# Nathan494326/Husky-Rover-MPPI-IsaacSim

Hardware: AMD Instinct MI355X
Metric: MPPI steps/sec at K=65536 H=100 on 750x750 costmap; 1/2/4/8-GPU scaling (higher is better)
Workload: dtype f32

## Files before the change

### husky-rover-mppi-isaacsim_amd/csrc/mppi_kernels.hip

```cpp
#include <hip/hip_runtime.h>

#include <algorithm>
#include <type_traits>
#include <stdint.h>

#include "mppi_detmath.h"
#include "mppi_kernels.h"

namespace mppi {

constexpr bool kFastMath = false;
constexpr bool kChainFast = true;

struct Recip {
  float b, y;
};
__device__ __forceinline__ bool div_ok(float v) {
  const float a = fabsf(v);
  return a >= 9.094947017729282e-13f && a <= 1.099511627776e12f;
}
template <bool F>
__device__ __forceinline__ Recip rc(float b, bool& bad) {
  Recip r;
  r.b = b;
// ... 330 lines not shown
}

struct Head {
  f2 xy;
  float z;
};

template <bool F>
__device__ __forceinline__ Head orient_step(f2 nxy, float nz, const Head& h, float sn, float cs, float omc,
                                           Lean& l) {
  const f2 hn = h.xy * nxy;
  const float d = (hn.x + hn.y) + h.z * nz;
  const f2 pxy = h.xy - bc2(d) * nxy;
  const float pz = h.z - d * nz;
  f2 txy, oxy;
  float tz, oz;
  if constexpr (F) {
    const f2 p2 = pxy * pxy;
    const Recip r = lean_norm2((p2.x + p2.y) + pz * pz, l);
    lean_div3<2>(pxy, pz, r, l, txy, tz);
    const f2 t2 = txy * txy;
    const Recip ro = norm_near1_trusted((t2.x + t2.y) + tz * tz);
    lean_div3<0>(txy, tz, ro, l, oxy, oz);
  } else {
    const float pn = sqrtf((pxy.x * pxy.x + pxy.y * pxy.y) + pz * pz);
    txy = f2{pxy.x / pn, pxy.y / pn};
    tz = pz / pn;
    const float tn = sqrtf((txy.x * txy.x + txy.y * txy.y) + tz * tz);
    oxy = f2{txy.x / tn, txy.y / tn};
    oz = tz / tn;
  }
  const f2 cxy = cross_xy(nxy, nz, oxy, oz);
  const f2 cz2 = nxy * oxy.yx;
  const float crz = cz2.x - cz2.y;
  const f2 no = nxy * oxy;
  const float dn = (no.x + no.y) + nz * oz;
  const f2 rxy = (oxy * bc2(cs) + cxy * bc2(sn)) + (nxy * bc2(dn)) * bc2(omc);
  const float rz = (oz * cs + crz * sn) + (nz * dn) * omc;
  Head o;
  if constexpr (F) {
    const f2 r2 = rxy * rxy;
    const Recip r = lean_norm_near1((r2.x + r2.y) + rz * rz, l);
    lean_div3<2>(rxy, rz, r, l, o.xy, o.z);
  } else {
    const float rn = sqrtf((rxy.x * rxy.x + rxy.y * rxy.y) + rz * rz);
    o.xy = f2{rxy.x / rn, rxy.y / rn};
    o.z = rz / rn;
  }
  return o;
}
template <bool F, bool GUARD = true>
__device__ __forceinline__ f2 advance_step(const Head& h, float v, float dt, f2 pos, Lean& l) {
  f2 u;
  if constexpr (F) {
    const f2 h2 = h.xy * h.xy;
    if constexpr (GUARD) {
      const Recip r = lean_norm_near1((h2.x + h2.y) + h.z * h.z, l);
      u = lean_div2(h.xy, r, l);
    } else {
      const Recip r = norm_near1_trusted((h2.x + h2.y) + h.z * h.z);
      u = lean_div2<0>(h.xy, r, l);
    }
  } else {
    const float hn = sqrtf((h.xy.x * h.xy.x + h.xy.y * h.xy.y) + h.z * h.z);
    u = f2{h.xy.x / hn, h.xy.y / hn};
  }
  return pos + (u * bc2(v)) * bc2(dt);
}

template <bool F>
__device__ __forceinline__ void wheels3d(const Dem& dem, float off, float x, float y,
                                         const float (&q)[4], float nx, float ny, float nz,
                                         float hx, float hy, float hz, StepOut& o, bool& bad) {
  o.z = bilinear<F>(x, y, q, dem.template rr<F>(), bad);
  const float cx = off * (ny * hz - nz * hy);
  const float cy = off * (nz * hx - nx * hz);
  o.lx = x + cx;
  o.ly = y + cy;
  o.lz = dem.template point<F>(o.lx, o.ly, bad);
  o.rx = x - cx;
  o.ry = y - cy;
  o.rz = dem.template point<F>(o.rx, o.ry, bad);
}

template <bool F>
__device__ __forceinline__ void step2d(const Dem& dem, float dt, float v, float sn, float cs,
                                       Traj& s, StepOut& o, bool& bad) {
  {
    const Recip r = rc<F>(sq<F>((s.hx * s.hx + s.hy * s.hy) + s.hz * s.hz, bad), bad);
    const float ux = dv<F>(s.hx, r, bad), uy = dv<F>(s.hy, r, bad);
    s.x = s.x + (ux * v) * dt;
    s.y = s.y + (uy * v) * dt;
  }
  {
    float nx = cs * s.hx - sn * s.hy;
    float ny = sn * s.hx + cs * s.hy;
    const float nrm = sq<F>(nx * nx + ny * ny, bad);
    if (nrm > 0.0f) {
      const Recip r = rc<F>(nrm, bad);
      nx = dv<F>(nx, r, bad);
      ny = dv<F>(ny, r, bad);
    }
    s.hx = nx;
    s.hy = ny;
    s.hz = 0.0f;
  }
  float q[4];
  dem.template corners<F>(s.x, s.y, q, bad);
  o.z = bilinear<F>(s.x, s.y, q, dem.template rr<F>(), bad);
  o.lx = o.ly = o.lz = o.rx = o.ry = o.rz = 0.0f;
}

template <bool F>
__device__ __forceinline__ float slope_term(float plx, float ply, float plz, float clx, float cly,
                                            float clz, float prx, float pry, float prz, float crx,
                                            float cry, float crz, bool& bad) {
  const float eps = 1e-6f;
  const float dzl = clz - plz;
  const float dxl = clx - plx, dyl = cly - ply;
  const float dl = sq<F>(dxl * dxl + dyl * dyl, bad);
  const float dzr = crz - prz;
  const float dxr = crx - prx, dyr = cry - pry;
  const float dr = sq<F>(dxr * dxr + dyr * dyr, bad);
  const float ratl = fabsf(dv1<F>(dzl, dl + eps, bad));
  const float ratr = fabsf(dv1<F>(dzr, dr + eps, bad));
  const float al = 1.0f + 5.0f * ratl;
  const float ar = 1.0f + 5.0f * ratr;
  const float ls = al * al, rs = ar * ar;
  return (ls > rs) ? ls : rs;
}

template <bool F>
__device__ __forceinline__ int costmap_index(int size, float hw, const Recip& rres_c, float x,
                                             float y, bool& bad, float rinv = 0.0f, int cdiv = 0) {
  float fx, fy;
  if (cdiv) {
    fx = cdiv_f(x + hw, rres_c.b, rinv);
    fy = cdiv_f((-y) + hw, rres_c.b, rinv);
  } else {
    fx = dv<F>(x + hw, rres_c, bad);
    fy = dv<F>((-y) + hw, rres_c, bad);
  }
  const int ix = (int)__builtin_amdgcn_fmed3f(fx, 0.0f, (float)(size - 1));
  const int iy = (int)__builtin_amdgcn_fmed3f(fy, 0.0f, (float)(size - 1));
  return ix + size * iy;
}


__device__ __forceinline__ float wave_min(float v) {
#pragma unroll
  for (int o = 32; o > 0; o >>= 1) v = fminf(v, __shfl_xor(v, o, 64));
  return v;
}

struct __attribute__((aligned(16))) PairScale {
  float m;
  float ea, eb;
  int mode;
};
__device__ __forceinline__ PairScale pair_scale(float ma, float mb, float T) {
  PairScale p;
  const bool ae = !(ma < INFINITY);
  const bool be = !(mb < INFINITY);
  p.m = fminf(ma, mb);
  p.ea = p.eb = 0.0f;
  if (ae) {
    p.mode = 2;
  } else if (be) {
    p.mode = 1;
  } else {
    p.mode = 0;
    p.ea = dm_expf(-((ma - p.m) / T));
    p.eb = dm_expf(-((mb - p.m) / T));
  }
  return p;
}
__device__ __forceinline__ double pair_apply(const PairScale& p, double a, double b, int j) {
  if (p.mode == 1) return a;
  if (p.mode == 2) return b;
  if (j == 0) return (double)p.m;
  return (double)p.ea * a + (double)p.eb * b;
}
__device__ __forceinline__ PairScale ld_scale(const PairScale* ps) { return *ps; }
__device__ __forceinline__ double pair_apply_raw(const PairScale p, double a, double b, int j) {
  double r = (double)p.ea * a + (double)p.eb * b;
  asm volatile("" : "+v"(r));
  const double n = j == 0 ? (double)p.m : r;
  return p.mode == 1 ? a : (p.mode == 2 ? b : n);
}
__device__ __forceinline__ double pair_apply_sel(const PairScale& ps, double a, double b, int j) {
  return pair_apply_raw(ps, a, b, j);
}

template <int G>
__device__ __forceinline__ void group_scales(const float (&m)[G], float T, PairScale (&ps)[G - 1]) {
  float cur[G];
#pragma unroll
  for (int i = 0; i < G; ++i) cur[i] = m[i];
  int base = 0;
#pragma unroll
  for (int w = G / 2; w >= 1; w >>= 1) {
#pragma unroll
    for (int i = 0; i < w; ++i) {
      ps[base + i] = pair_scale(cur[2 * i], cur[2 * i + 1], T);
      cur[i] = ps[base + i].m;
    }
    base += w;
  }
}
template <int G>
__device__ __forceinline__ double group_apply(const PairScale* ps, const double (&v)[G], int j) {
  double cur[G];
#pragma unroll
  for (int i = 0; i < G; ++i) cur[i] = v[i];
  int base = 0;
#pragma unroll
  for (int w = G / 2; w >= 1; w >>= 1) {
#pragma unroll
    for (int i = 0; i < w; ++i) cur[i] = pair_apply(ps[base + i], cur[2 * i], cur[2 * i + 1], j);
    base += w;
  }
  return cur[0];
}

template <bool FRESH, int NT = 1024>
__device__ __forceinline__ int thread_id() {
  int t = threadIdx.x;
  if constexpr (FRESH) asm volatile("" : "+v"(t));
  __builtin_assume(t >= 0 && t < NT);
  return t;
}

struct NoiseVals {
  float a1, a2, b1, b2;
};
__device__ __forceinline__ NoiseVals noise_gen(uint64_t seed, uint64_t n_base, int64_t k_offset, int blk, int n, int tj) {
  const uint64_t kg = (uint64_t)(k_offset + (int64_t)blk * 256 + tj);
  NoiseVals v;
  noise_block_pk(seed, n_base + (uint64_t)n, kg, &v.a1, &v.a2, &v.b1, &v.b2);
  return v;
}
__device__ __forceinline__ void noise_store(float* __restrict__ eps, int H, int blk, int n, int tj, const NoiseVals& v) {
  const int t = 2 * n;
  float* e1 = eps + ((size_t)blk * 2 * H + t) * 256 + tj;
  float* e2 = e1 + (size_t)H * 256;
  __hip_atomic_store(e1, v.a1, __ATOMIC_RELAXED, __HIP_MEMORY_SCOPE_AGENT);
  __hip_atomic_store(e2, v.a2, __ATOMIC_RELAXED, __HIP_MEMORY_SCOPE_AGENT);
  if (t + 1 < H) {
    __hip_atomic_store(e1 + 256, v.b1, __ATOMIC_RELAXED, __HIP_MEMORY_SCOPE_AGENT);
    __hip_atomic_store(e2 + 256, v.b2, __ATOMIC_RELAXED, __HIP_MEMORY_SCOPE_AGENT);
  }
}
__device__ __forceinline__ void noise_unit(uint64_t seed, uint64_t n_base, int64_t k_offset, int H, int blk, int n,
                                           float* __restrict__ eps, int tj) {
  noise_store(eps, H, blk, n, tj, noise_gen(seed, n_base, k_offset, blk, n, tj));
}
__device__ __forceinline__ void noise_rows(uint64_t seed, uint64_t n_base, int64_t k_offset, int H, int end,
                                           float* __restrict__ eps, int g0, int gstride, int tj) {
  const int NB = (H + 1) >> 1;
  if (g0 >= end) return;
  int blk = g0 / NB, n = g0 - blk * NB;
  const int sq = gstride / NB, sr = gstride - sq * NB;
  for (int g = g0; g < end; g += gstride) {
    noise_unit(seed, n_base, k_offset, H, blk, n, eps, tj);
    blk += sq;
    n += sr;
    if (n >= NB) {
      n -= NB;
      ++blk;
    }
  }
}
struct NoisePos {
  int q, g, blk, n;
};
__device__ __forceinline__ void noise_pos_step(NoisePos& p, int stride, int NB) {
  p.q += stride;
  p.n += (p.q >> 2) - p.g;
  p.g = p.q >> 2;
  while (p.n >= NB) {
    p.n -= NB;
    ++p.blk;
  }
}
__device__ __forceinline__ void noise_waves(uint64_t seed, uint64_t n_base, int64_t k_offset, int H, int q, int q1,
                                            int stride, float* __restrict__ eps, int lane) {
  const int NB = (H + 1) >> 1;
  if (q >= q1) return;
  NoisePos a;
  a.q = q;
  a.g = q >> 2;
  a.blk = a.g / NB;
  a.n = a.g - a.blk * NB;
  for (;;) {
    NoisePos b = a;
    noise_pos_step(b, stride, NB);
    const bool has_b = b.q < q1;
    if (!has_b) b = a;
    const NoiseVals va = noise_gen(seed, n_base, k_offset, a.blk, a.n, ((a.q & 3) << 6) + lane);
    const NoiseVals vb = noise_gen(seed, n_base, k_offset, b.blk, b.n, ((b.q & 3) << 6) + lane);
    noise_store(eps, H, a.blk, a.n, ((a.q & 3) << 6) + lane, va);
    if (!has_b) break;
    noise_store(eps, H, b.blk, b.n, ((b.q & 3) << 6) + lane, vb);
    a = b;
    noise_pos_step(a, stride, NB);
    if (a.q >= q1) break;
  }
}

constexpr int UCACHE_ROW = 256 + 4;
template <int TB, int NT, bool EPS = false, bool WT = false>
__device__ __forceinline__ void leaf_records(const RolloutArgs& a, const float* cost_lds,
                                             unsigned char* scratch, const float* ub_block,
                                             const float* unom = nullptr, const float* ucache = nullptr,
                                             int uc_steps = 0, int blk = -1);

template <int TB, int NT, bool EPS, bool WT>
__device__ __forceinline__ void leaf_records(const RolloutArgs& a, const float* cost_lds,
                                             unsigned char* scratch, const float* ub_block,
                                             const float* unom, const float* ucache, int uc_steps, int blk) {
  if (blk < 0) blk = blockIdx.x;
  constexpr int NL = TB / 256;
  constexpr int NWL = TB / 64;
  const int tid = thread_id<WT, NT>(), lane = tid & 63;
  const int wave = __builtin_amdgcn_readfirstlane(tid >> 6);
  const int H = a.H, E = 2 * H + 2;
  float* wbuf = reinterpret_cast<float*>(scratch);
  float* wave_m = wbuf + TB;
  double* red = reinterpret_cast<double*>(scratch + ((TB + NWL) * 4 + 15) / 16 * 16);
  const int NR = NL * (E - 1);
  const int NU = ((NR + 7) >> 3) << 6;
  struct Unit {
    float4 uq[8];
    int j;
    bool cached;
    float nom, sg, lo, hi;
    const float4* w4;
  };
  auto load = [&](int it, Unit& U) __attribute__((always_inline)) {
    const int k = (it >> 3) & 7;
    const int r = min(((it >> 6) << 3) + (it & 7), NR - 1);
    const int half = k >> 2, line = k & 3;
    const int leaf = r / (E - 1), j = 1 + r - leaf * (E - 1);
    U.j = j;
    const int tr0 = 256 * leaf + 128 * half + 32 * line;
    U.w4 = reinterpret_cast<const float4*>(wbuf + tr0);
    const float4* u4 = reinterpret_cast<const float4*>(ub_block + (size_t)(j >= 2 ? j - 2 : 0) * TB + tr0);
    U.cached = false;
    U.nom = U.sg = U.lo = U.hi = 0.f;
    if constexpr (EPS) {
      const int c = (j - 2) >= H ? 1 : 0;
      const int t = max(j - 2, 0) - c * H;
      const int ti = min(t + 1, H - 1);
      U.nom = unom[c * H + ti];
      U.sg = c ? a.s2 : a.s1;
      U.lo = c ? a.min_u2 : a.min_u1;
      U.hi = c ? a.max_u2 : a.max_u1;
      if (j >= 2 && t < uc_steps) {
        U.cached = true;
        u4 = reinterpret_cast<const float4*>(ucache + (size_t)(c * uc_steps + t) * UCACHE_ROW + tr0);
      }
    }
#pragma unroll
    for (int g = 0; g < 8; ++g) U.uq[g] = (j >= 2) ? u4[g] : make_float4(1.f, 1.f, 1.f, 1.f);
  };
  auto reduce = [&](int it, const Unit& U) __attribute__((always_inline)) {
    const int j = U.j;
    double gs[8];
#pragma unroll
    for (int g = 0; g < 8; ++g) {
      const float4 w = U.w4[g];
      float4 u = U.uq[g];
      if (EPS && !U.cached) {
        u.x = clampf(U.nom + U.sg * u.x, U.lo, U.hi);
        u.y = clampf(U.nom + U.sg * u.y, U.lo, U.hi);
        u.z = clampf(U.nom + U.sg * u.z, U.lo, U.hi);
        u.w = clampf(U.nom + U.sg * u.w, U.lo, U.hi);
      }
      if (j < 2) u = make_float4(1.f, 1.f, 1.f, 1.f);
      const double x = __builtin_fma((double)w.x, (double)u.x, (double)w.y * (double)u.y);
      const double y = __builtin_fma((double)w.z, (double)u.z, (double)w.w * (double)u.w);
      gs[g] = x + y;
    }
    const double ls = ((gs[0] + gs[1]) + (gs[2] + gs[3])) + ((gs[4] + gs[5]) + (gs[6] + gs[7]));
    const double s2 = ls + __shfl_xor(ls, 8, 64);
    const double hs = s2 + __shfl_xor(s2, 16, 64);
    const double rs = hs + __shfl_xor(hs, 32, 64);
    const int r = ((it >> 6) << 3) + (it & 7);
    if (r < NR && ((it >> 3) & 7) == 0) {
      const int leaf = r / (E - 1);
      red[leaf * E + j] = rs;
    }
  };
  Unit first;
  if (tid < NU) load(tid, first);
  if (wave < NWL) {
    const float wm = wave_min(cost_lds[tid]);
    if (lane == 0) wave_m[wave] = wm;
  }
  __syncthreads();
  for (int j = tid; j < TB; j += NT) {
    const int leaf = j >> 8;
    const float m = fminf(fminf(wave_m[4 * leaf], wave_m[4 * leaf + 1]),
                          fminf(wave_m[4 * leaf + 2], wave_m[4 * leaf + 3]));
    const float c = cost_lds[j];
    wbuf[j] = (c < INFINITY) ? dm_expf(-((c - m) / a.T)) : 0.0f;
  }
  __syncthreads();
  if (tid < NU) reduce(tid, first);
  for (int it = NT + tid; it < NU; it += NT) {
    Unit U;
    load(it, U);
    reduce(it, U);
  }
  __syncthreads();
  for (int j = tid; j < E; j += NT) {
    double val[NL];
    float lm[NL];
#pragma unroll
    for (int q = 0; q < NL; ++q) {
      lm[q] = fminf(fminf(wave_m[4 * q], wave_m[4 * q + 1]), fminf(wave_m[4 * q + 2], wave_m[4 * q + 3]));
      val[q] = (j == 0) ? (double)lm[q] : red[q * E + j];
    }
#pragma unroll
    for (int width = NL; width > 1; width >>= 1) {
#pragma unroll
      for (int q = 0; q < width / 2; ++q) {
        const PairScale ps = pair_scale(lm[2 * q], lm[2 * q + 1], a.T);
        val[q] = pair_apply(ps, val[2 * q], val[2 * q + 1], j);
        lm[q] = ps.m;
      }
    }
    if constexpr (WT)
      __hip_atomic_store(a.nodes + (size_t)blk * E + j, val[0], __ATOMIC_RELAXED, __HIP_MEMORY_SCOPE_AGENT);
    else
      a.nodes[(size_t)blk * E + j] = val[0];
    if (j == 0 && a.rec_m) {
      if constexpr (WT)
        __hip_atomic_store(a.rec_m + blk, lm[0], __ATOMIC_RELAXED, __HIP_MEMORY_SCOPE_AGENT);
      else
        a.rec_m[blk] = lm[0];
    }
  }
}

constexpr int PAIR_D = PAIR_RING;
constexpr int PAIR_LAG = 4;
static_assert(PAIR_LAG > 0 && PAIR_LAG < PAIR_D, "ring depth must exceed the consume lag");
static_assert(PAIR_LAG % 2 == 0, "the side loop pairs even and odd steps");

__device__ __forceinline__ int lds_load_acquire(const int* f) {
  const int v = __hip_atomic_load(f, __ATOMIC_RELAXED, __HIP_MEMORY_SCOPE_WORKGROUP);
  __builtin_amdgcn_fence(__ATOMIC_ACQUIRE, "workgroup", "local");
  return v;
}
__device__ __forceinline__ void lds_store_release(int* f, int v) {
  __builtin_amdgcn_fence(__ATOMIC_RELEASE, "workgroup", "local");
  __hip_atomic_store(f, v, __ATOMIC_RELAXED, __HIP_MEMORY_SCOPE_WORKGROUP);
}

__device__ __forceinline__ void lds_wait_ge(const int* f, int target, int& seen) {
  if (seen >= target) return;
  int v;
  while ((v = lds_load_acquire(f)) < target) {
  }
  seen = v;
}

template <int TB, int NC, bool DUMP, int DO = PAIR_D>
__device__ __forceinline__ void chain_wave_3d(const RolloutArgs& a, const Dem& dem, const Traj& s, int tj,
                                              bool valid, int64_t kl, const float* ring_in, float* ring_out,
                                              const int* f_prod, int* f_chain, const int* const (&f_cons)[NC],
                                              int& seen_prod, int (&seen_cons)[NC]) {
  constexpr int D = PAIR_D;
  constexpr int RI = 4;
  using T_ = std::true_type;
  using F_ = std::false_type;
  const int H = a.H;
  bool nobad = false;
  const bool clk = a.clk != nullptr && blockIdx.x == 0 && tj < 64;
  uint64_t clk_t0 = 0, clk_r0 = 0;
  if (clk) {
    clk_t0 = __builtin_amdgcn_s_memtime();
    clk_r0 = __builtin_amdgcn_s_memrealtime();
  }
  auto body = [&](auto cd_tag) __attribute__((always_inline)) {
      constexpr bool CD = decltype(cd_tag)::value;
      Head hd{f2{s.hx, s.hy}, s.hz};
      f2 posA = f2{s.x, s.y}, posB = posA;
      float4 nvA = make_float4(0.f, 0.f, 0.f, 0.f), nvB = nvA;
      float snA = 0.f, csA = 0.f, omA = 0.f, snB = 0.f, csB = 0.f, omB = 0.f;
      const f2 cell_off = f2{-a.x_min, a.y_min};
      const float fi_hi = (float)(a.grid - 1), fj_lo = (float)(1 - a.rows);
      const char* nbase = reinterpret_cast<const char*>(dem.N);
      const int nrow = a.grid + 1;
      const int ncol0 = a.grid + 2;
      auto gather = [&](f2 pos, float4& nv) __attribute__((always_inline)) {
        f2 f;
        if constexpr (CD) {
          const f2 aa = pos + cell_off;
          const f2 q0 = aa * bc2(dem.rinv);
          const f2 r = pk_fma(-q0, bc2(dem.res), aa);
          f = pk_fma(r, bc2(dem.rinv), q0);
        } else {
          f = f2{(pos.x - a.x_min) / a.res, (pos.y + a.y_min) / a.res};
        }
        const int ti = (int)__builtin_amdgcn_fmed3f(f.x, -1.0f, fi_hi);
        const int tjj = (int)__builtin_amdgcn_fmed3f(f.y, fj_lo, 1.0f);
        const int idx = __mul24(tjj, -nrow) + (ti + ncol0);
        nv = *reinterpret_cast<const float4*>(nbase + (uint32_t)(idx << 4));
      };
      auto read_in = [&](int t, float& v, float& sn, float& cs, float& om, int need) __attribute__((always_inline)) {
        if (need) lds_wait_ge(f_prod, need, seen_prod);
        const float* ri = ring_in + (t % D) * RI * TB + tj;
        v = ri[0];
        sn = ri[TB];
        cs = ri[2 * TB];
        om = ri[3 * TB];
      };
      {
        float v0;
        read_in(0, v0, snA, csA, omA, 1);
        Lean l;
        lean_init(l);
        f2 p = advance_step<true>(hd, v0, a.dt, posA, l);
        if (__builtin_expect(lean_bad(l), 0)) p = advance_step<false>(hd, v0, a.dt, posA, l);
        posA = p;
        gather(posA, nvA);
      }
      auto it = [&](auto even_tag, auto more_tag, int t, f2& pX, float4& nX, float& snX, float& csX, float& omX,
                    f2& pY, float4& nY, float& snY, float& csY, float& omY) __attribute__((always_inline)) {
        constexpr bool EVEN = decltype(even_tag)::value;
        constexpr bool more = decltype(more_tag)::value;
        float v1 = 0.f;
        if constexpr (more) read_in(t + 1, v1, snY, csY, omY, EVEN ? min(t + 3, H) : 0);
        const f2 nxy = f2{nX.x, nX.y};
        const float nz = nX.z;
        Lean l;
        lean_init(l);
        Head ho = orient_step<true>(nxy, nz, hd, snX, csX, omX, l);
        f2 p1 = pX;
        if constexpr (more) p1 = advance_step<true, false>(ho, v1, a.dt, pX, l);
        if (__builtin_expect(lean_bad(l), 0)) {
          ho = orient_step<false>(nxy, nz, hd, snX, csX, omX, l);
          if constexpr (more) p1 = advance_step<false>(ho, v1, a.dt, pX, l);
        }
        const f2 cxy = bc2(a.off) * cross_xy(nxy, nz, ho.xy, ho.z);
        if constexpr (more) {
          pY = p1;
          gather(pY, nY);
        }
        if constexpr (EVEN) {
#pragma unroll
          for (int c = 0; c < NC; ++c) lds_wait_ge(f_cons[c], t - DO + 2, seen_cons[c]);
        }
        float* ro = ring_out + (t % DO) * 4 * TB + tj;
        ro[0] = pX.x;
        ro[TB] = pX.y;
        ro[2 * TB] = cxy.x;
        ro[3 * TB] = cxy.y;
        if constexpr (DUMP) {
          if (valid) {
            float q[4];
            dem.template corners<false>(pX.x, pX.y, q, nobad);
            const float z = bilinear<false>(pX.x, pX.y, q, dem.template rr<false>(), nobad);
            const size_t o3 = ((size_t)kl * H + t) * 3;
// ... 1839 lines not shown
    bool flagged = false;
    if (what == 0) {
      const float want = a / b;
      const float got = dv1<true>(a, b, flagged);
      if (!flagged && f_bits(want) != f_bits(got)) ++local;
    } else if (what == 1) {
      const float x = fabsf(a);
      const float want = sqrtf(x);
      const float got = sq<true>(x, flagged);
      if (!flagged && f_bits(want) != f_bits(got)) ++local;
    } else {
      const U4 r2 = philox4x32_10(U4{(uint32_t)i, (uint32_t)(i >> 32), 0x5e1fu, 0x1ea4u}, (uint32_t)seed,
                                  (uint32_t)(seed >> 32));
      const float c = (what == 3) ? bits_f((r2.x & 0x807FFFFFu) | ((127u - 30u + r2.y % 60u) << 23))
                                  : mk(r2.x, r2.y);
      const float n = (a * a + b * b) + c * c;
      const float sr = sqrtf(n);
      Lean l;
      lean_init(l);
      const Recip rr = lean_norm(n, l);
      const float g0 = lean_div(a, rr, l), g1 = lean_div(b, rr, l), g2 = lean_div(c, rr, l);
      if (!lean_bad(l) && (f_bits(rr.b) != f_bits(sr) || f_bits(g0) != f_bits(a / sr) ||
                           f_bits(g1) != f_bits(b / sr) || f_bits(g2) != f_bits(c / sr)))
        ++local;
    }
  }
  if (local) atomicAdd(bad_count, local);
}

template <int TB, int PROJ>
static hipError_t launch_pair_m(const RolloutArgs& a, int blocks, size_t lds, hipStream_t st, int mode,
                                bool dump) {
  if (mode == 0) {
    if (dump)
      hipLaunchKernelGGL((mppi_rollout_pair_kernel<TB, PROJ, 0, true>), dim3(blocks), dim3(2 * TB), lds, st, a);
    else
      hipLaunchKernelGGL((mppi_rollout_pair_kernel<TB, PROJ, 0, false>), dim3(blocks), dim3(2 * TB), lds, st, a);
  } else {
    if (dump)
      hipLaunchKernelGGL((mppi_rollout_pair_kernel<TB, PROJ, 1, true>), dim3(blocks), dim3(2 * TB), lds, st, a);
    else
      hipLaunchKernelGGL((mppi_rollout_pair_kernel<TB, PROJ, 1, false>), dim3(blocks), dim3(2 * TB), lds, st, a);
  }
  return hipGetLastError();
}

template <int TB, int PROJ>
static hipError_t launch_roles_m(const RolloutArgs& a, int blocks, size_t lds, hipStream_t st, int mode,
                                 bool dump) {
  const dim3 g(blocks), b(NROLES * TB);
  if (mode == 0) {
    if (dump)
      hipLaunchKernelGGL((mppi_rollout_roles_kernel<TB, PROJ, 0, true>), g, b, lds, st, a);
    else
      hipLaunchKernelGGL((mppi_rollout_roles_kernel<TB, PROJ, 0, false>), g, b, lds, st, a);
  } else {
    if (dump)
      hipLaunchKernelGGL((mppi_rollout_roles_kernel<TB, PROJ, 1, true>), g, b, lds, st, a);
    else
      hipLaunchKernelGGL((mppi_rollout_roles_kernel<TB, PROJ, 1, false>), g, b, lds, st, a);
  }
  return hipGetLastError();
}

hipError_t launch_rollout_pair(const RolloutArgs& a, int blocks, size_t lds, hipStream_t st, int proj,
                               int mode, bool dump, bool roles) {
  if (roles) {
    if (proj == 3) return launch_roles_m<256, 3>(a, blocks, lds, st, mode, dump);
    return launch_roles_m<256, 2>(a, blocks, lds, st, mode, dump);
  }
  if (proj == 3) return launch_pair_m<256, 3>(a, blocks, lds, st, mode, dump);
  return launch_pair_m<256, 2>(a, blocks, lds, st, mode, dump);
}

hipError_t launch_finish(const FinishArgs& f, size_t lds, hipStream_t st, int groups) {
  hipLaunchKernelGGL(mppi_finish_kernel, dim3(groups), dim3(FIN_THREADS), lds, st, f);
  return hipGetLastError();
}

int colfin_shape(int n, int H, int* P_out, int* ncol_out, int* groups_out, size_t* lds_tree, int max_groups) {
  if (n < 1 || n > COLFIN_PMAX || max_groups < 1) return 0;
  int P = 16;
  while (P < n) P *= 2;
  const int E = 2 * H + 2;
  const int ncol = std::max({2, (E + 63) / 64, (E + max_groups - 1) / max_groups});
  if ((ncol + 1) * (P / 16) > FIN_THREADS) return 0;
  const int groups = (E + ncol - 1) / ncol;
  *P_out = P;
  *ncol_out = ncol;
  *groups_out = groups;
  *lds_tree = (size_t)(P - 1) * sizeof(PairScale) + (size_t)(2 * P) * sizeof(float) +
              (size_t)(ncol + 1) * (P / 16) * sizeof(double);
  return 1;
}

hipError_t launch_colfin(const FinishArgs& f, size_t lds, hipStream_t st, int P, int ncol, int groups) {
  hipLaunchKernelGGL(mppi_colfin_kernel, dim3(groups), dim3(FIN_THREADS), lds, st, f, P, ncol);
  return hipGetLastError();
}

hipError_t launch_tail(const FinishArgs& f, hipStream_t st) {
  const size_t lds = (size_t)(12 * f.H + 4) * sizeof(float);
  hipLaunchKernelGGL(mppi_tail_kernel, dim3(1), dim3(TAIL_THREADS), lds, st, f);
  return hipGetLastError();
}

__global__ __launch_bounds__(256) void mppi_normal_table_kernel(const float* __restrict__ Z, int rows, int grid,
                                                                float res, float4* __restrict__ out) {
  const int64_t cols = (int64_t)grid + 1;
  const int64_t n = ((int64_t)rows + 1) * cols;
  const float res_half_neg = (-res) / 2.0f;
  const float res_sq = res * res;
  for (int64_t g = (int64_t)blockIdx.x * 256 + threadIdx.x; g < n; g += (int64_t)gridDim.x * 256) {
    const int j = (int)(g / cols) - 1, i = (int)(g % cols) - 1;
    const int r0 = clampi(j, 0, rows - 1), r1 = clampi(j + 1, 0, rows - 1);
    const int c0 = clampi(i, 0, grid - 1), c1 = clampi(i + 1, 0, grid - 1);
    const float q0 = Z[(size_t)r0 * grid + c0], q1 = Z[(size_t)r0 * grid + c1];
    const float q2 = Z[(size_t)r1 * grid + c0], q3 = Z[(size_t)r1 * grid + c1];
    bool unused = false;
    const float vx = res_half_neg * (((q1 - q0) - q2) + q3);
    const float vy = res_half_neg * (((q2 - q0) - q1) + q3);
    const Recip r = rc<false>(sq<false>((vx * vx + vy * vy) + res_sq * res_sq, unused), unused);
    out[g] = make_float4(dv<false>(vx, r, unused), dv<false>(vy, r, unused), dv<false>(res_sq, r, unused), 0.0f);
  }
}

hipError_t launch_normal_table(const float* Z, int rows, int grid, float res, float4* out, hipStream_t st) {
  const int64_t n = ((int64_t)rows + 1) * ((int64_t)grid + 1);
  const unsigned blocks = (unsigned)std::min<int64_t>((n + 255) / 256, 256 * 16);
  hipLaunchKernelGGL(mppi_normal_table_kernel, dim3(blocks), dim3(256), 0, st, Z, rows, grid, res, out);
  return hipGetLastError();
}

__global__ __launch_bounds__(256) void mppi_noise_kernel(uint64_t seed, uint64_t n_base, int64_t k_offset,
                                                         int H, int n_blocks, float* __restrict__ eps) {
  noise_rows(seed, n_base, k_offset, H, n_blocks * ((H + 1) >> 1), eps, blockIdx.x, gridDim.x, threadIdx.x);
}

struct ServerLaunch {
  RolloutArgs a;
  ServerArgs z;
};
__device__ __forceinline__ const ServerLaunch* fresh_args() {
#if __HIP_DEVICE_COMPILE__
  uint64_t v = reinterpret_cast<uint64_t>(__builtin_amdgcn_kernarg_segment_ptr());
  asm volatile("" : "+s"(v));
  return (const ServerLaunch*)reinterpret_cast<const __attribute__((address_space(4))) ServerLaunch*>(v);
#else
  return nullptr;
#endif
}

template <int TB, int PROJ>
__global__ __launch_bounds__(NROLES * TB) void mppi_step_server_kernel(const ServerLaunch args) {
  __shared__ unsigned cmd_lds[32];
  __shared__ int sh[2];
  const int tid = threadIdx.x;
  unsigned expect = args.z.first_seq;
  bool head = blockIdx.x == 0;
  for (;;) {
    const auto* L = fresh_args();
    const ServerArgs& z = L->z;
    if (tid < 64) {
      const int slot = tid < kCmdWords ? tid : 0;
      const unsigned long long* src =
          (head ? reinterpret_cast<const unsigned long long*>(z.cmd->slot) : z.relay) + slot;
      const unsigned* host_stop = reinterpret_cast<const unsigned*>(z.cmd->slot + kCmdStopSlot);
      unsigned ok = 0;
      unsigned long long w = 0;
      const uint64_t t0 = __builtin_amdgcn_s_memrealtime();
      uint64_t t_stop = t0;
      if (tid == 0 && head && z.clk) z.clk[kClkServer + 8 * (expect & 7) + 6] = t0;
      const bool forced = head && z.exit_after != 0 && expect - z.first_seq >= z.exit_after;
      while (!forced) {
        w = head ? __hip_atomic_load(src, __ATOMIC_RELAXED, __HIP_MEMORY_SCOPE_SYSTEM)
                 : __hip_atomic_load(src, __ATOMIC_RELAXED, __HIP_MEMORY_SCOPE_AGENT);
        const unsigned lo = (unsigned)w, hi = (unsigned)(w >> 32);
        const unsigned long long stop_slot = (unsigned)__builtin_amdgcn_readlane((int)lo, kCmdStopSlot);
        if (cmd_stop_hit(stop_slot, z.launch_id)) break;
        const unsigned seq0 = (unsigned)__builtin_amdgcn_readfirstlane((int)hi);
        if (__builtin_amdgcn_ballot_w64(!cmd_slot_ok(slot, w, seq0, expect)) == 0) {
          ok = 1;
          break;
        }
        const uint64_t now = __builtin_amdgcn_s_memrealtime();
        if (head) {
          if (now - t0 >= z.idle_ticks) break;
        } else {
          if (now - t_stop >= 10000) {
            t_stop = now;
            if (__hip_atomic_load(host_stop, __ATOMIC_RELAXED, __HIP_MEMORY_SCOPE_SYSTEM) == z.launch_id) break;
          }
          __builtin_amdgcn_s_sleep(2);
        }
      }
      if (ok && tid < kCmdWords) {
        if (head && tid != kCmdStopSlot)
          __hip_atomic_store(z.relay + tid, w, __ATOMIC_RELAXED, __HIP_MEMORY_SCOPE_AGENT);
        cmd_lds[tid] = (unsigned)w;
      }
      if (head && !ok && tid == 0)
        __hip_atomic_store(z.relay + kCmdStopSlot, (unsigned long long)z.launch_id, __ATOMIC_RELAXED,
                           __HIP_MEMORY_SCOPE_AGENT);
      if (tid == 0) cmd_lds[31] = ok;
      if (tid == 0 && head && z.clk && ok)
        __hip_atomic_store(z.clk + kClkServer + 8 * (cmd_lds[0] & 7), (uint64_t)__builtin_amdgcn_s_memrealtime(),
                           __ATOMIC_RELAXED, __HIP_MEMORY_SCOPE_AGENT);
    }
    __syncthreads();
    if (!cmd_lds[31]) return;
    const ServerCmd& c = *reinterpret_cast<const ServerCmd*>(cmd_lds);
    auto rd = [&](const float& x) __attribute__((always_inline)) {
      return __builtin_bit_cast(float, __builtin_amdgcn_readfirstlane(__builtin_bit_cast(int, x)));
    };
    const unsigned seq = __builtin_amdgcn_readfirstlane(c.seq);
    const int eps_slot = __builtin_amdgcn_readfirstlane(c.eps_slot);
    const int cur = __builtin_amdgcn_readfirstlane(c.cur);
    RolloutArgs a = L->a;
    a.eps = z.eps[eps_slot];
    a.u_nom1 = z.u_nom[cur];
    a.u_nom2 = z.u_nom[cur] + a.H;
    a.x0 = rd(c.x0);
    a.y0 = rd(c.y0);
    a.h0x = rd(c.h0x);
    a.h0y = rd(c.h0y);
    a.h0z = rd(c.h0z);
    a.wl = rd(c.wl);
    a.wr = rd(c.wr);
    a.gx = rd(c.gx);
    a.gy = rd(c.gy);
    a.s1 = rd(c.s1);
    a.s2 = rd(c.s2);
    a.igx = rd(c.igx);
    a.igy = rd(c.igy);
    a.pf_scale = rd(c.pf_scale);
    a.pf_far = __builtin_amdgcn_readfirstlane(c.pf_far);
    a.speed_on = __builtin_amdgcn_readfirstlane(c.speed_on);
    const int nslot = __builtin_amdgcn_readfirstlane(c.noise_slot);
    const uint64_t nbase = ((uint64_t)__builtin_amdgcn_readfirstlane(c.noise_n_base_hi) << 32) |
                           (uint32_t)__builtin_amdgcn_readfirstlane(c.noise_n_base_lo);
    const int64_t W = 4 * (int64_t)z.nroll * ((a.H + 1) >> 1);
    const int nn = z.nroll - z.fin_groups;
    const int64_t S = 2 * (int64_t)nn + z.fin_groups - 1;
    const int ticket = roles_body<TB, PROJ, 0, false, true>(a, (int)blockIdx.x, z.rec_cnt, sh);
    if (ticket == z.nroll - 1 && tid == 0 && z.clk) {
      const uint64_t now = __builtin_amdgcn_s_memrealtime();
      z.clk[kClkServer + 8 * (seq & 7) + 1] = now;
      const uint64_t t0 = __hip_atomic_load(z.clk + kClkServer + 8 * (seq & 7), __ATOMIC_RELAXED, __HIP_MEMORY_SCOPE_AGENT);
      __hip_atomic_fetch_add(z.clk + kClkSums, now - t0, __ATOMIC_RELAXED, __HIP_MEMORY_SCOPE_AGENT);
      __hip_atomic_fetch_add(z.clk + kClkSums + 1, (uint64_t)1, __ATOMIC_RELAXED, __HIP_MEMORY_SCOPE_AGENT);
    }
    const int blk = ticket - (z.nroll - z.fin_groups);
    if (blk < 0 && nslot >= 0) {
      __builtin_amdgcn_s_setprio(0);
      const int wave = __builtin_amdgcn_readfirstlane(tid >> 6);
      const int q0 = (int)(W * (2 * ticket) / S), q1 = (int)(W * (2 * ticket + 2) / S);
      noise_waves(a.seed, nbase, a.k_offset, a.H, q0 + wave, q1, NROLES * TB / 64, z.eps[nslot], tid & 63);
    }
    if (blk >= 0) {
      __builtin_amdgcn_s_setprio(0);
      if (tid == 0) {
        const uint64_t t0 = __builtin_amdgcn_s_memrealtime();
        int late = z.wait_ticks == 0;
        while (!late && ticket != z.nroll - 1 &&
               __hip_atomic_load(z.rec_cnt, __ATOMIC_RELAXED, __HIP_MEMORY_SCOPE_AGENT) < (unsigned)z.nroll) {
          if (__builtin_amdgcn_s_memrealtime() - t0 >= z.wait_ticks ||
              __hip_atomic_load(z.f.abort, __ATOMIC_RELAXED, __HIP_MEMORY_SCOPE_AGENT) == seq) {
            late = 1;
            break;
          }
          __builtin_amdgcn_s_sleep(2);
        }
        if (late) __hip_atomic_store(z.f.abort, seq, __ATOMIC_RELAXED, __HIP_MEMORY_SCOPE_AGENT);
        sh[1] = late;
      }
      __syncthreads();
      bool ok = !sh[1];
      if (ok) {
        FinishArgs f = z.f;
        const int mode = __builtin_amdgcn_readfirstlane(c.mode);
        const int slot = __builtin_amdgcn_readfirstlane(c.tail_slot);
        f.mode = mode;
        f.seq = seq;
        f.u_nom_next = z.u_nom[cur ^ 1];
        f.tail_in = z.tail_in[slot];
        f.tail_out = z.tail_out[slot];
        f.x0 = a.x0;
        f.y0 = a.y0;
        f.h0x = a.h0x;
        f.h0y = a.h0y;
        f.h0z = a.h0z;
        f.wl = a.wl;
        f.wr = a.wr;
        ok = colfin_body<true>(f, z.fin_P, z.fin_ncol, blk, z.fin_groups, z.rec_cnt);
        if (ok && blk == z.fin_groups - 1 && tid == 0 && z.clk) {
          const uint64_t now = __builtin_amdgcn_s_memrealtime();
          z.clk[kClkServer + 8 * (seq & 7) + 2] = now;
          const uint64_t t0 = __hip_atomic_load(z.clk + kClkServer + 8 * (seq & 7), __ATOMIC_RELAXED, __HIP_MEMORY_SCOPE_AGENT);
          __hip_atomic_fetch_add(z.clk + kClkSums + 2, now - t0, __ATOMIC_RELAXED, __HIP_MEMORY_SCOPE_AGENT);
          __hip_atomic_fetch_add(z.clk + kClkSums + 3, (uint64_t)1, __ATOMIC_RELAXED, __HIP_MEMORY_SCOPE_AGENT);
        }
      }
      if (!ok && tid == 0)
        __hip_atomic_store(z.f.done, seq | kDoneFail, __ATOMIC_RELAXED, __HIP_MEMORY_SCOPE_SYSTEM);
      if (nslot >= 0 && blk < z.fin_groups - 1) {
        const int wave = __builtin_amdgcn_readfirstlane(tid >> 6);
        const int q0 = (int)(W * (2 * nn + blk) / S), q1 = (int)(W * (2 * nn + blk + 1) / S);
// ... 78 lines not shown
```

Before: 12630.

## Skip zero-weight lines in leaf weighted-sum reduction via ballot liveness masks

```diff
diff --git a/husky-rover-mppi-isaacsim_amd/csrc/mppi_kernels.hip b/husky-rover-mppi-isaacsim_amd/csrc/mppi_kernels.hip
--- a/husky-rover-mppi-isaacsim_amd/csrc/mppi_kernels.hip
+++ b/husky-rover-mppi-isaacsim_amd/csrc/mppi_kernels.hip
@@ -506,6 +506,9 @@
   for (int o = 32; o > 0; o >>= 1) v = fminf(v, __shfl_xor(v, o, 64));
   return v;
 }
+__device__ __forceinline__ float uniform_f(float v) {
+  return __builtin_bit_cast(float, __builtin_amdgcn_readfirstlane(__builtin_bit_cast(int, v)));
+}
 
 struct __attribute__((aligned(16))) PairScale {
   float m;
@@ -688,84 +691,184 @@
     float4 uq[8];
     int j;
     bool cached;
-    float nom, sg, lo, hi;
-    const float4* w4;
+    int c;
+    float nom;
+    int tr0;
   };
-  auto load = [&](int it, Unit& U) __attribute__((always_inline)) {
-    const int k = (it >> 3) & 7;
-    const int r = min(((it >> 6) << 3) + (it & 7), NR - 1);
-    const int half = k >> 2, line = k & 3;
+  auto load = [&](int r, int k, unsigned gm, Unit& U) __attribute__((always_inline)) {
     const int leaf = r / (E - 1), j = 1 + r - leaf * (E - 1);
     U.j = j;
-    const int tr0 = 256 * leaf + 128 * half + 32 * line;
-    U.w4 = reinterpret_cast<const float4*>(wbuf + tr0);
+    const int tr0 = 256 * leaf + 32 * k;
+    U.tr0 = tr0;
     const float4* u4 = reinterpret_cast<const float4*>(ub_block + (size_t)(j >= 2 ? j - 2 : 0) * TB + tr0);
     U.cached = false;
-    U.nom = U.sg = U.lo = U.hi = 0.f;
+    U.nom = 0.f;
+    U.c = 0;
     if constexpr (EPS) {
       const int c = (j - 2) >= H ? 1 : 0;
       const int t = max(j - 2, 0) - c * H;
       const int ti = min(t + 1, H - 1);
       U.nom = unom[c * H + ti];
-      U.sg = c ? a.s2 : a.s1;
-      U.lo = c ? a.min_u2 : a.min_u1;
-      U.hi = c ? a.max_u2 : a.max_u1;
+      U.c = c;
       if (j >= 2 && t < uc_steps) {
         U.cached = true;
         u4 = reinterpret_cast<const float4*>(ucache + (size_t)(c * uc_steps + t) * UCACHE_ROW + tr0);
       }
     }
 #pragma unroll
-    for (int g = 0; g < 8; ++g) U.uq[g] = (j >= 2) ? u4[g] : make_float4(1.f, 1.f, 1.f, 1.f);
+    for (int g = 0; g < 8; ++g) U.uq[g] = (j >= 2 && ((gm >> g) & 1u)) ? u4[g] : make_float4(1.f, 1.f, 1.f, 1.f);
   };
-  auto reduce = [&](int it, const Unit& U) __attribute__((always_inline)) {
+  auto line_sum = [&](const Unit& U, unsigned gm) __attribute__((always_inline)) {
     const int j = U.j;
+    const float4* w4 = reinterpret_cast<const float4*>(wbuf + U.tr0);
+    const float sg = U.c ? a.s2 : a.s1;
+    const float lo = U.c ? a.min_u2 : a.min_u1;
+    const float hi = U.c ? a.max_u2 : a.max_u1;
     double gs[8];
 #pragma unroll
     for (int g = 0; g < 8; ++g) {
-      const float4 w = U.w4[g];
+      if (!((gm >> g) & 1u)) {
+        gs[g] = 0.0;
+        continue;
+      }
+      const float4 w = w4[g];
       float4 u = U.uq[g];
       if (EPS && !U.cached) {
-        u.x = clampf(U.nom + U.sg * u.x, U.lo, U.hi);
-        u.y = clampf(U.nom + U.sg * u.y, U.lo, U.hi);
-        u.z = clampf(U.nom + U.sg * u.z, U.lo, U.hi);
-        u.w = clampf(U.nom + U.sg * u.w, U.lo, U.hi);
+        u.x = clampf(U.nom + sg * u.x, lo, hi);
+        u.y = clampf(U.nom + sg * u.y, lo, hi);
+        u.z = clampf(U.nom + sg * u.z, lo, hi);
+        u.w = clampf(U.nom + sg * u.w, lo, hi);
       }
       if (j < 2) u = make_float4(1.f, 1.f, 1.f, 1.f);
       const double x = __builtin_fma((double)w.x, (double)u.x, (double)w.y * (double)u.y);
       const double y = __builtin_fma((double)w.z, (double)u.z, (double)w.w * (double)u.w);
       gs[g] = x + y;
     }
-    const double ls = ((gs[0] + gs[1]) + (gs[2] + gs[3])) + ((gs[4] + gs[5]) + (gs[6] + gs[7]));
+    return ((gs[0] + gs[1]) + (gs[2] + gs[3])) + ((gs[4] + gs[5]) + (gs[6] + gs[7]));
+  };
+  auto dense_load = [&](int it, Unit& U) __attribute__((always_inline)) {
+    load(min(((it >> 6) << 3) + (it & 7), NR - 1), (it >> 3) & 7, 0xffu, U);
+  };
+  auto dense_reduce = [&](int it, const Unit& U) __attribute__((always_inline)) {
+    const double ls = line_sum(U, 0xffu);
     const double s2 = ls + __shfl_xor(ls, 8, 64);
     const double hs = s2 + __shfl_xor(s2, 16, 64);
     const double rs = hs + __shfl_xor(hs, 32, 64);
     const int r = ((it >> 6) << 3) + (it & 7);
     if (r < NR && ((it >> 3) & 7) == 0) {
       const int leaf = r / (E - 1);
-      red[leaf * E + j] = rs;
+      red[leaf * E + U.j] = rs;
     }
   };
-  Unit first;
-  if (tid < NU) load(tid, first);
-  if (wave < NWL) {
-    const float wm = wave_min(cost_lds[tid]);
-    if (lane == 0) wave_m[wave] = wm;
-  }
-  __syncthreads();
-  for (int j = tid; j < TB; j += NT) {
-    const int leaf = j >> 8;
-    const float m = fminf(fminf(wave_m[4 * leaf], wave_m[4 * leaf + 1]),
-                          fminf(wave_m[4 * leaf + 2], wave_m[4 * leaf + 3]));
-    const float c = cost_lds[j];
-    wbuf[j] = (c < INFINITY) ? dm_expf(-((c - m) / a.T)) : 0.0f;
-  }
-  __syncthreads();
-  if (tid < NU) reduce(tid, first);
-  for (int it = NT + tid; it < NU; it += NT) {
-    Unit U;
-    load(it, U);
-    reduce(it, U);
+  float lmin[NL];
+  bool early = true;
+#pragma unroll
+  for (int q = 0; q < NL; ++q) {
+    const float4 c4 = reinterpret_cast<const float4*>(cost_lds + 256 * q)[lane];
+    const float c = fminf(fminf(c4.x, c4.y), fminf(c4.z, c4.w));
+    const float lo = uniform_f(wave_min(c));
+    lmin[q] = lo;
+    const unsigned long long near = __ballot(c < INFINITY && !(-((c - lo) / a.T) < -87.0f));
+    unsigned long long lines = near | (near >> 4);
+    lines |= lines >> 2;
+    lines |= lines >> 1;
+    early = early && (lines & 0x0101010101010101ull) == 0x0101010101010101ull;
+  }
+  auto weights = [&](auto mask_tag) __attribute__((always_inline)) {
+    for (int j = tid; j < TB; j += NT) {
+      const int leaf = j >> 8;
+      float m = lmin[0];
+#pragma unroll
+      for (int q = 1; q < NL; ++q) m = (leaf == q) ? lmin[q] : m;
+      const float c = cost_lds[j];
+      const float w = (c < INFINITY) ? dm_expf(-((c - m) / a.T)) : 0.0f;
+      wbuf[j] = w;
+      if constexpr (!decltype(mask_tag)::value) continue;
+      unsigned long long gb = __ballot(w != 0.0f);
+      gb |= gb >> 1;
+      gb = (gb | (gb >> 2)) & 0x1111111111111111ull;
+      gb = (gb | (gb >> 3)) & 0x0303030303030303ull;
+      gb = (gb | (gb >> 6)) & 0x000f000f000f000full;
+      gb = (gb | (gb >> 12)) & 0x000000ff000000ffull;
+      gb = (gb | (gb >> 24)) & 0xffffull;
+      if (lane == 0) reinterpret_cast<unsigned short*>(red + leaf * E)[(j >> 6) & 3] = (unsigned short)gb;
+    }
+    if (tid < NWL) {
+      float m = lmin[0];
+#pragma unroll
+      for (int q = 1; q < NL; ++q) m = ((tid >> 2) == q) ? lmin[q] : m;
+      wave_m[tid] = m;
+    }
+  };
+  auto dense_rounds = [&](int it0) __attribute__((always_inline)) {
+    for (int it = it0 + tid; it < NU; it += NT) {
+      Unit U;
+      dense_load(it, U);
+      dense_reduce(it, U);
+    }
+  };
+  if (early) {
+    Unit first;
+    if (tid < NU) dense_load(tid, first);
+    weights(std::false_type{});
+    __syncthreads();
+    if (tid < NU) dense_reduce(tid, first);
+    dense_rounds(NT);
+  } else {
+    weights(std::true_type{});
+    __syncthreads();
+    unsigned long long live = 0ull;
+    bool all_lines = true;
+#pragma unroll
+    for (int q = 0; q < NL; ++q) {
+      const unsigned long long gq = *reinterpret_cast<const unsigned long long*>(red + q * E);
+      live |= gq;
+      unsigned long long t = gq | (gq >> 4);
+      t |= t >> 2;
+      t |= t >> 1;
+      all_lines = all_lines && (t & 0x0101010101010101ull) == 0x0101010101010101ull;
+    }
+    live = ((unsigned long long)(unsigned)__builtin_amdgcn_readfirstlane((int)(live >> 32)) << 32) |
+           (unsigned)__builtin_amdgcn_readfirstlane((int)live);
+    if (all_lines) {
+      dense_rounds(0);
+    } else {
+      const int r = wave * 64 + lane;
+      if (r < NR) {
+        unsigned long long todo = live;
+        double rs;
+        for (;;) {
+          double l0 = 0.0, p0 = 0.0, h0 = 0.0;
+          rs = 0.0;
+#pragma clang loop unroll(disable)
+          for (int k = 0; k < 8; ++k) {
+            const unsigned gm = (unsigned)(todo >> (8 * k)) & 0xffu;
+            double s = 0.0;
+            if (gm) {
+              Unit U;
+              load(r, k, gm, U);
+              s = line_sum(U, gm);
+            }
+            if (!(k & 1)) {
+              l0 = s;
+            } else {
+              const double p = l0 + s;
+              if (!(k & 2)) {
+                p0 = p;
+              } else {
+                const double h = p0 + p;
+                if (!(k & 4)) h0 = h;
+                else rs = h0 + h;
+              }
+            }
+          }
+          if (todo == ~0ull || !(rs == 0.0)) break;
+          todo = ~0ull;
+        }
+        const int leaf = r / (E - 1);
+        red[leaf * E + (1 + r - leaf * (E - 1))] = rs;
+      }
+    }
   }
   __syncthreads();
   for (int j = tid; j < E; j += NT) {
@@ -2911,7 +3014,8 @@
 }
 
 template <int TB, int PROJ>
-__global__ __launch_bounds__(NROLES * TB) void mppi_step_server_kernel(const ServerLaunch args) {
+__global__ __launch_bounds__(NROLES * TB) __attribute__((amdgpu_num_vgpr(56))) void mppi_step_server_kernel(
+    const ServerLaunch args) {
   __shared__ unsigned cmd_lds[32];
   __shared__ int sh[2];
   const int tid = threadIdx.x;
diff --git a/profiles/leaf_dense_timing.py b/profiles/leaf_dense_timing.py
--- /dev/null
+++ b/profiles/leaf_dense_timing.py
@@ -0,0 +1,61 @@
+#!/usr/bin/env python3
+import argparse
+import json
+import os
+import sys
+import time
+
+ROOT = os.path.dirname(os.path.dirname(os.path.abspath(__file__)))
+sys.path[:0] = [ROOT, os.path.join(ROOT, "husky-rover-mppi-isaacsim_amd")]
+
+
+def main():
+    ap = argparse.ArgumentParser()
+    ap.add_argument("--temperature", type=float, default=3000.0)
+    ap.add_argument("--steps", type=int, default=200)
+    ap.add_argument("--warmup", type=int, default=20)
+    ap.add_argument("--reps", type=int, default=5)
+    ap.add_argument("-K", type=int, default=65536)
+    ap.add_argument("-H", type=int, default=100)
+    args = ap.parse_args()
+    from mppi_amd import _lib, scene
+
+    Z, hw, cm = scene.scene_c3()
+    eng = _lib.Engine(_lib.make_params(args.K, args.H, temperature=args.temperature), 0)
+    eng.set_dem(Z, hw)
+    eng.set_costmap(cm, hw)
+    eng.set_state(_lib.make_state(-60.0, -5.0, (1.0, 0.0, 0.0), goal_x=65.0, goal_y=10.0))
+    eng.set_async_tail(True)
+    runs = []
+    step = 0
+    try:
+        for _ in range(args.warmup):
+            eng.step("3d", step, copy=False)
+            step += 1
+        for _ in range(args.reps):
+            eng.outputs()
+            eng.sync()
+            t0 = time.perf_counter()
+            for _ in range(args.steps):
+                eng.step("3d", step, copy=False)
+                step += 1
+            eng.outputs()
+            eng.sync()
+            runs.append((time.perf_counter() - t0) / args.steps * 1e6)
+        r_us, s_us, n = eng.server_time()
+        info = eng.launch_info()
+    finally:
+        eng.close()
+    runs_sorted = sorted(runs)
+    print(json.dumps(dict(temperature=args.temperature, K=args.K, H=args.H, steps=args.steps,
+                          us_per_step=[round(x, 2) for x in runs],
+                          median_us=round(runs_sorted[len(runs) // 2], 2),
+                          spread_us=round(runs_sorted[-1] - runs_sorted[0], 2),
+                          server_rollout_us=round(r_us / n, 2) if n else None,
+                          server_step_us=round(s_us / n, 2) if n else None,
+                          resident=info["resident"], server_launches=info["server_launches"],
+                          lib=os.environ.get("MPPI_LIB_PATH") or "default")))
+
+
+if __name__ == "__main__":
+    main()
```

New measurement: 12960 (median of 6 runs). 1.03x the previous value.
